# JanWosnitza/FrayTracer

Hardware: AMD Instinct MI355X
Metric: Mrays/s (primary+secondary) at 4096x4096; max per-pixel |delta| vs F# ref (delta is measured against the CPU oracle: F# parity is unpinned, DESIGN.md section 2) (higher is better)
Workload: dtype f32

## Files before the change

fraytracer_amd/_lib.py:

```python
import ctypes as C
import os

_HERE = os.path.dirname(os.path.abspath(__file__))
LIB_PATH = os.environ.get("FRAYTRACER_HIP_LIB") or os.path.join(_HERE, "libfraytracer_hip.so")

FT_OPT_REFILL_MIN, FT_OPT_MAX_BLOCKS_PER_CU, FT_OPT_HOST_CHUNKS, FT_OPT_HOST_PIN, FT_OPT_TAIL_K, FT_OPT_MATH, FT_OPT_GUIDED, FT_OPT_CHUNK, FT_OPT_CULL, FT_OPT_ESCAPE, FT_OPT_LAZY_UNION, FT_OPT_CARVED, FT_OPT_REUSE, FT_OPT_CERT, FT_OPT_CERT_POLICY, FT_OPT_ORDER, FT_OPT_OCCL, FT_OPT_OCCL_POLICY = 1, 2, 3, 4, 5, 6, 7, 8, 9, 10, 11, 12, 13, 14, 15, 16, 17, 18
FT_MATH_FIXED, FT_MATH_GLIBC_FMA, FT_MATH_GLIBC_SSE2 = 0, 1, 2
FT_OK, FT_ERR_INVALID, FT_ERR_NO_DEVICE, FT_ERR_HIP, FT_ERR_UNSUPPORTED, FT_ERR_EMPTY, FT_ERR_COMM = 0, -1, -2, -3, -4, -5, -6


class FrayTracerError(RuntimeError):
    def __init__(self, code, message):
        super().__init__(f"libfraytracer_hip error {code}: {message}")
        self.code = code


class Vec3(C.Structure):
    _fields_ = [("x", C.c_float), ("y", C.c_float), ("z", C.c_float)]


class Ray(C.Structure):
    _fields_ = [("origin", Vec3), ("direction", Vec3), ("length", C.c_float), ("epsilon", C.c_float)]


class Boundary(C.Structure):
    _fields_ = [("center", Vec3), ("radius", C.c_float)]


class Sphere(C.Structure):
# ... 245 lines not shown
```

fraytracer_amd/api.py:

```python
import contextlib
import ctypes as C
import threading

import numpy as np

from . import _lib
from ._lib import lib, check, FrayTracerError


def _v3(v):
    x, y, z = (float(np.float32(c)) for c in v)
    return (x, y, z)


class FColor(tuple):

    @staticmethod
    def ofRGB(r, g, b):
        return FColor(_v3((r, g, b)))


class _Desc:
    __slots__ = ("kind", "args", "kids", "__weakref__")

# ... 337 lines not shown
    @contextlib.contextmanager
    def on_current_stream(self, tensor):
        import torch
        cur = torch.cuda.current_stream(tensor.device)
        side = None
        if int(cur.cuda_stream) == 0:
            side = self._side_stream = getattr(self, "_side_stream", None) or torch.cuda.Stream(tensor.device)
            side.wait_stream(cur)
        handle = int((side or cur).cuda_stream)
        if getattr(self, "_adopted", None) != handle:
            self.set_stream(handle)
        try:
            yield
        finally:
            if side is not None:
                cur.wait_stream(side)

    OPTIONS = {"refill_min": _lib.FT_OPT_REFILL_MIN, "max_blocks_per_cu": _lib.FT_OPT_MAX_BLOCKS_PER_CU,
               "host_chunks": _lib.FT_OPT_HOST_CHUNKS, "host_pin": _lib.FT_OPT_HOST_PIN, "math": _lib.FT_OPT_MATH,
               "tail_k": _lib.FT_OPT_TAIL_K, "guided": _lib.FT_OPT_GUIDED, "chunk": _lib.FT_OPT_CHUNK, "cull": _lib.FT_OPT_CULL, "escape": _lib.FT_OPT_ESCAPE, "lazy_union": _lib.FT_OPT_LAZY_UNION, "carved": _lib.FT_OPT_CARVED, "reuse": _lib.FT_OPT_REUSE,
               "cert": _lib.FT_OPT_CERT, "cert_policy": _lib.FT_OPT_CERT_POLICY,
               "order": _lib.FT_OPT_ORDER,
               "occl": _lib.FT_OPT_OCCL, "occl_policy": _lib.FT_OPT_OCCL_POLICY}

    def set_option(self, name, value):
        check(lib.ft_ctx_set_option(self._ctx, self._option_id(name), int(value)))

    def get_option(self, name):
        v = C.c_int32()
        check(lib.ft_ctx_get_option(self._ctx, self._option_id(name), C.byref(v)))
        return int(v.value)

    def _option_id(self, name):
        return self.OPTIONS[name]

    def sphere(self, c, r): return check(lib.ft_form_sphere(self._ctx, C.byref(_lib.Sphere(_vec(c), r))))
    def capsule(self, a, b, r): return check(lib.ft_form_capsule(self._ctx, C.byref(_lib.Capsule(_vec(a), _vec(b), r))))
    def torus(self, c, n, R, r): return check(lib.ft_form_torus(self._ctx, C.byref(_lib.Torus(_vec(c), _vec(n), R, r))))
    def triangle(self, a, b, c, r): return check(lib.ft_form_triangle(self._ctx, C.byref(_lib.Triangle(_vec(a), _vec(b), _vec(c), r))))
    def box(self, c, h): return check(lib.ft_form_box(self._ctx, C.byref(_lib.Box(_vec(c), _vec(h)))))
    def form_union(self, hs): return check(lib.ft_form_union(self._ctx, *_handles(hs)))
    def form_subtract(self, a, b): return check(lib.ft_form_subtract(self._ctx, a, b))
    def form_intersect(self, hs): return check(lib.ft_form_intersect(self._ctx, *_handles(hs)))
    def form_union_smooth(self, k, hs): return check(lib.ft_form_union_smooth(self._ctx, k, *_handles(hs)))
    def material_solid(self, rgb): return check(lib.ft_material_solid(self._ctx, _f3(rgb)))
    def material_glass(self, tint, ior, dispersion): return check(lib.ft_material_glass(self._ctx, _f3(tint), ior, dispersion))
    def object_create(self, m, f): return check(lib.ft_object_create(self._ctx, m, f))
    def object_union(self, hs): return check(lib.ft_object_union(self._ctx, *_handles(hs)))
    def object_subtract(self, o, f): return check(lib.ft_object_subtract(self._ctx, o, f))
    def object_intersect(self, o, hs): return check(lib.ft_object_intersect(self._ctx, o, *_handles(hs)))
    def light_directional(self, d, c): return check(lib.ft_light_directional(self._ctx, _f3(d), _f3(c)))
    def light_point(self, p, c): return check(lib.ft_light_point(self._ctx, _f3(p), _f3(c)))

    def form_boundary(self, h):
        b = _lib.Boundary()
        check(lib.ft_form_boundary(self._ctx, h, C.byref(b)))
        return (b.center.x, b.center.y, b.center.z, b.radius)
# ... 1042 lines not shown
```

fraytracer_amd/csrc/capi.cpp:

```cpp
#include <hip/hip_runtime_api.h>

#include <algorithm>
#include <atomic>
#include <array>
#include <cmath>
#include <cstdlib>
#include <cstring>
#include <string>
#include <vector>

#include "../../include/fraytracer_hip.h"
#include "build_hash.h"
#include "ft_kernels.h"
#include "ft_mesh.h"
#include "ft_slice.h"
#include "ft_refine.h"
#include "ft_shells.h"
#include "ft_measure.h"
#include "scene.hpp"

#ifndef FT_BUILD_KIND
#define FT_BUILD_KIND "product"
#endif

// ... 29 lines not shown
    std::vector<hipEvent_t> syncEvents;
    std::vector<std::pair<void*, size_t>> hostRegs;
    std::vector<std::pair<hipEvent_t, hipEvent_t>> events;
    std::vector<std::pair<hipEvent_t, hipEvent_t>> eventPool;
    double foldedMs = 0.0;
    int optRefillMin = 64;
    int optMaxBlocksPerCU = 0;
    int optHostChunks = 0;
    int optHostPin = 1;
    int optMath = FT_MATH_FIXED;
    int optTailK = -1;
    int optChunk = 64;
    int optEscape = 1;
    int optLazyUnion = 1;
    int optCull = 1;
    int optReuse = 1;
    int optCarved = 1;
    int optCert = 1;
    int optCertPolicy = 0;
    int optGuided = 0;
    int optOccl = 1;
    int optOcclPolicy = 0;
    int optOrder = 1;
    int fieldBrick = -1;
    uint32_t meshTile = FT_MESH_TILE_DEFAULT;
    uint32_t sliceTile = FT_SLICE_TILE_DEFAULT;
    int sliceStop = 0;
    int64_t sliceLast[2] = {0, 0};
    void* sliceWork = nullptr; size_t sliceWorkBytes = 0;
    void* refineWork = nullptr; size_t refineWorkBytes = 0;
    uint32_t shellsTile = FT_SHELLS_TILE_DEFAULT;
    int shellsStop = 0;
    int64_t shellsLast[2] = {0, 0};
    void* shellsWork = nullptr; size_t shellsWorkBytes = 0;
    void* measureWork = nullptr; size_t measureWorkBytes = 0;
    int measureStop = 0, measureEager = 0;
    unsigned measureGrid = 0;
    int refineSkipField = 0;
    uint32_t orderNum = 1, orderDen = 1;
};

struct TileOrderKey {
    int32_t W, H, x0, nCols;
    uint32_t stripeW, stripeRanks, stripeRank, nJobs, variant, libm;
    bool operator==(const TileOrderKey& o) const {
        return W == o.W && H == o.H && x0 == o.x0 && nCols == o.nCols && stripeW == o.stripeW && stripeRanks == o.stripeRanks && stripeRank == o.stripeRank &&
               nJobs == o.nJobs && variant == o.variant && libm == o.libm;
    }
};
struct TileOrderSlot {
    uint32_t* cost = nullptr; uint32_t* order = nullptr; void* work = nullptr;
    uint32_t capTiles = 0;
    bool keyed = false, hasOrder = false;
    bool usedOrder = false;
    TileOrderKey key{};
};

struct ft_scene {
    ft_ctx* ctx = nullptr;
    ft::FlatScene flat;
    void* dBlob = nullptr;
    FtSceneDev dev{};
    const float* dMaterialsExt = nullptr;
    const int32_t* dMatHandles = nullptr;
    FtCarve carve{};
    bool usesExpLog = false;
    mutable TileOrderSlot orderSlots[2];
};

namespace {

int requireDevice(ft_ctx* c) {
    if (!c) return setErr(FT_ERR_INVALID, "null context");
    if (!c->hasDevice) return setErr(FT_ERR_NO_DEVICE, "context has no GPU: libfraytracer_hip has no CPU fallback");
    hipError_t e = hipSetDevice(c->device);
    if (e != hipSuccess) return hipFail(e, "hipSetDevice");
// ... 155 lines not shown
    hipEvent_t e0, e1;
    if ((rc = acquireEvents(c, e0, e1))) return rc;
    const char* at = "hipEventRecord";
    hipError_t e = hipEventRecord(e0, stream);
    if (e == hipSuccess && (e = launch()) != hipSuccess) at = what;
    if (e == hipSuccess) e = hipEventRecord(e1, stream);
    if (e != hipSuccess) { c->eventPool.emplace_back(e0, e1); return hipFail(e, at); }
    c->events.emplace_back(e0, e1);
    return FT_OK;
}

int clampPerCU(const ft_ctx* c, const char* kernel, int& perCU) {
    if (perCU < 1) return setErr(FT_ERR_UNSUPPORTED, std::string("the ") + kernel + " kernel does not fit a compute unit with this scene's LDS footprint");
    perCU = std::min(perCU, 8);
    if (c->optMaxBlocksPerCU > 0) perCU = std::min(perCU, c->optMaxBlocksPerCU);
    return FT_OK;
}

TileOrderSlot* tileOrderSlot(const ft_scene* s, int lane, uint32_t nTiles) {
    TileOrderSlot& t = s->orderSlots[lane];
    if (t.capTiles >= nTiles) return &t;
    if (t.cost) (void)hipFree(t.cost);
    t = TileOrderSlot{};
    const size_t words = 2 * (size_t)nTiles, bytes = align256(words * sizeof(uint32_t)) + ft_tile_order_work_bytes(nTiles);
    void* p = nullptr;
    if (hipMalloc(&p, bytes) != hipSuccess) { (void)hipGetLastError(); return nullptr; }
    t.cost = static_cast<uint32_t*>(p);
    t.order = t.cost + nTiles;
    t.work = static_cast<unsigned char*>(p) + align256(words * sizeof(uint32_t));
    t.capTiles = nTiles;
    return &t;
}


int gridSize(const ft_ctx* c, const FtTraceKey& key, const KernelPlan& plan, uint32_t nJobs, unsigned& blocks) {
    int perCU = 0;
    HIP_TRY(ft_trace_occupancy(key, plan.lds, &perCU));
    int rc = clampPerCU(c, "trace", perCU); if (rc) return rc;
    if (c->optMaxBlocksPerCU <= 0 && key.variant != 1u) {
        const uint64_t tiles = ((uint64_t)nJobs + (uint64_t)c->optChunk - 1) / (uint64_t)c->optChunk;
        const uint64_t wavesPerLayer = (uint64_t)c->numCUs * (FT_BLOCK / 64);
        const uint64_t want = (tiles + 2 * wavesPerLayer) / (4 * wavesPerLayer);
        perCU = (int)std::min<uint64_t>((uint64_t)perCU, std::max<uint64_t>(2, want));
    }
    const uint64_t maxBlocks = (uint64_t)c->numCUs * perCU;
    const uint64_t wantBlocks = ((uint64_t)nJobs + FT_BLOCK - 1) / FT_BLOCK;
    blocks = (unsigned)std::max<uint64_t>(1, std::min(maxBlocks, wantBlocks));
    return FT_OK;
}

void handOut(const ft_ctx* c, const ft_scene* s, unsigned variant, unsigned blocks, FtRenderArgs& a) {
// ... 23 lines not shown
    a.bundlePeriod = pol.bundle == 0u ? FT_BUNDLE_PERIOD : pol.bundle == 3u ? 0u : pol.bundle;
    a.bundleMin = pol.bundle == 0u ? FT_BUNDLE_MIN : 1u;
    a.bundleShadow = pol.bundle == 0u ? FT_BUNDLE_SHADOW : pol.bundle == 2u ? 2u : 0u;
    if (c->optCertPolicy == 0 && a.cert && a.mode == 0u && a.views == nullptr && a.maxSize > 0.0f) {
        const float* cm = a.cam;
        const double dx = (double)cm[0] - f.hdr.escC[0], dy = (double)cm[1] - f.hdr.escC[1], dz = (double)cm[2] - f.hdr.escC[2];
        auto len = [cm](int i) { return std::sqrt((double)cm[i] * cm[i] + (double)cm[i + 1] * cm[i + 1] + (double)cm[i + 2] * cm[i + 2]); };
        const double up = len(6), rt = len(9), fw = len(3);
        const double reach = std::sqrt(dx * dx + dy * dy + dz * dz) + (double)f.hdr.escR;
        const double tile = 8.0 * std::max(up, rt) / (double)a.maxSize * reach / fw;
        if (fw > 0.0 && tile <= (double)f.hdr.certM) a.certPrim = a.certShadow = 0xffffffffu;
    }
}

void occlSchedule(const ft_ctx* c, const ft::FlatScene& f, FtRenderArgs& a) {
    const OcclPolicy pol = decodeOcclPolicy((uint32_t)c->optOcclPolicy);
    const bool on = a.cert && c->optOccl && f.occ.b >= 0.0f && pol.period != 255u;
    a.occPeriod = on ? (pol.period != 0u ? pol.period : FT_OCCL_PERIOD) : 0u;
    a.occFrom = pol.from + a.reuse;
    a.occMin = pol.minLanes != 0u ? pol.minLanes : FT_OCCL_MIN;
    a.occ = f.occ;
}

TileOrderSlot* tileOrder(const ft_ctx* c, const ft_scene* s, int lane, const FtTraceKey& key, FtRenderArgs& a) {
    a.tileCost = nullptr; a.tileOrder = nullptr;
    TileOrderSlot* slot = nullptr;
    if (key.form == FT_FORM_FRAME && !key.ext && key.variant == 1u && a.mode == 0u && a.spp == 1u && a.chunk == 64u && a.refillMin == 64u && !c->optGuided && a.shrink1 == a.nJobs && a.nJobs >= 64u) {
        if (c->optOrder == 0) { s->orderSlots[lane].keyed = s->orderSlots[lane].hasOrder = s->orderSlots[lane].usedOrder = false; }
        else slot = tileOrderSlot(s, lane, a.nJobs >> 6);
    }
    if (slot) {
        const TileOrderKey k{a.W, a.H, a.x0, a.nCols, a.stripeW, a.stripeRanks, a.stripeRank, a.nJobs, key.variant, key.libm ? 1u : 0u};
        a.tileCost = slot->cost;
        if (c->optOrder == 1 && slot->keyed && slot->hasOrder && slot->key == k) a.tileOrder = slot->order;
        slot->key = k; slot->keyed = true; slot->hasOrder = false; slot->usedOrder = a.tileOrder != nullptr;
    }
    return slot;
}

int launchTrace(ft_ctx* c, const ft_scene* s, FtRenderArgs& a, int lane = 0) {
    hipStream_t stream = lane ? c->lane1 : c->stream;
    uint32_t* counter = c->dCounter + (lane ? 16 : 0);
    KernelPlan plan;
    int rc = planTrace(c, s, a.ext != 0u, a.shade, plan); if (rc) return rc;
    a.S = s->dev; a.S.fastPath = plan.variant; a.S.nSlots = plan.nSlots;
    a.S.mathFma = c->optMath == FT_MATH_GLIBC_FMA ? 1u : 0u;
    if (!c->optEscape) a.S.escR = -1.0f;
    a.carve = s->carve; a.materialsExt = s->dMaterialsExt;
    a.math = plan.libm ? 1u : 0u;
    a.counter = counter; a.stats = c->dStats;
    a.cull = (s->dev.cullPc != 0xffffffffu && plan.cullRows && c->optCull) ? 1u : 0u;
    a.lazy = c->optLazyUnion ? 1u : 0u;
    a.reuse = (c->optReuse && !a.shade) ? 1u : 0u;
    const FtTraceKey key = ft_trace_key(a);
    unsigned blocks = 0;
    if ((rc = gridSize(c, key, plan, a.nJobs, blocks))) return rc;
    handOut(c, s, plan.variant, blocks, a);
    certSchedule(c, s->flat, plan.variant, a);
// ... 8 lines not shown
    return FT_OK;
}

struct OptionSpec { int32_t id; int ft_ctx::*field; int32_t lo, hi; const char* err; };
constexpr OptionSpec kOptions[] = {
    {FT_OPT_REFILL_MIN, &ft_ctx::optRefillMin, 1, 64, "FT_OPT_REFILL_MIN: 1 .. 64"},
    {FT_OPT_MAX_BLOCKS_PER_CU, &ft_ctx::optMaxBlocksPerCU, 0, 8, "FT_OPT_MAX_BLOCKS_PER_CU: 0 (no cap) .. 8"},
    {FT_OPT_HOST_CHUNKS, &ft_ctx::optHostChunks, 0, 16, "FT_OPT_HOST_CHUNKS: 0 (automatic) .. 16"},
    {FT_OPT_HOST_PIN, &ft_ctx::optHostPin, 0, 1, "FT_OPT_HOST_PIN: 0 or 1"},
    {FT_OPT_TAIL_K, &ft_ctx::optTailK, -1, 64, "FT_OPT_TAIL_K: -1 (default), 0 (off) .. 64"},
    {FT_OPT_MATH, &ft_ctx::optMath, FT_MATH_FIXED, FT_MATH_GLIBC_SSE2, "FT_OPT_MATH: 0 fixed, 1 glibc (FMA build), 2 glibc (SSE2 build)"},
    {FT_OPT_GUIDED, &ft_ctx::optGuided, 0, 1, "FT_OPT_GUIDED: 0 or 1"},
    {FT_OPT_CHUNK, &ft_ctx::optChunk, 16, 64, "FT_OPT_CHUNK: 64, 32 or 16"},
    {FT_OPT_CULL, &ft_ctx::optCull, 0, 1, "FT_OPT_CULL: 0 or 1"},
    {FT_OPT_ESCAPE, &ft_ctx::optEscape, 0, 1, "FT_OPT_ESCAPE: 0 or 1"},
    {FT_OPT_LAZY_UNION, &ft_ctx::optLazyUnion, 0, 1, "FT_OPT_LAZY_UNION: 0 or 1"},
    {FT_OPT_CARVED, &ft_ctx::optCarved, 0, 1, "FT_OPT_CARVED: 0 or 1"},
    {FT_OPT_REUSE, &ft_ctx::optReuse, 0, 1, "FT_OPT_REUSE: 0 or 1"},
    {FT_OPT_CERT, &ft_ctx::optCert, 0, 1, "FT_OPT_CERT: 0 or 1"},
    {FT_OPT_CERT_POLICY, &ft_ctx::optCertPolicy, INT32_MIN, INT32_MAX, "FT_OPT_CERT_POLICY: 0, or bits 16-23 (due lanes) in 1 .. 64"},
    {FT_OPT_ORDER, &ft_ctx::optOrder, 0, 2, "FT_OPT_ORDER: 0 off, 1 heavy tiles first, 2 record only"},
    {FT_OPT_OCCL, &ft_ctx::optOccl, 0, 1, "FT_OPT_OCCL: 0 or 1"},
    {FT_OPT_OCCL_POLICY, &ft_ctx::optOcclPolicy, 0, 0x40ffff, "FT_OPT_OCCL_POLICY: 0, or bits 0-7 period, 8-15 first step, 16-23 candidates (0 .. 64)"},
};
const OptionSpec* findOption(int32_t id) {
    for (const OptionSpec& o : kOptions) if (o.id == id) return &o;
    return nullptr;
}
bool optionAccepts(const OptionSpec& o, int32_t v) {
    if (v < o.lo || v > o.hi) return false;
    if (o.id == FT_OPT_CHUNK) return v == 64 || v == 32 || v == 16;
    if (o.id == FT_OPT_CERT_POLICY) { const uint32_t mn = decodeCertPolicy((uint32_t)v).minLanes; return v == 0 || (mn >= 1u && mn <= 64u); }
    return true;
}

int checkJobCount(uint64_t views, uint64_t samples, const ft_render_params* p) {
    const uint64_t tiles = (uint64_t)((p->n_columns + 7) / 8) * (uint64_t)((p->height + 7) / 8);
    if (views * samples * tiles * 64 >= 0xFFFF0000ull) return setErr(FT_ERR_UNSUPPORTED, "more than 2^32 samples in one call");
    return FT_OK;
}

int checkParams(const ft_render_params* p) {
    if (!p) return setErr(FT_ERR_INVALID, "null render params");
    if (p->width <= 0 || p->height <= 0 || p->n_columns <= 0) return setErr(FT_ERR_INVALID, "empty image");
    if (p->stripe_width <= 0 || p->stripe_ranks <= 0 || p->stripe_rank < 0 || p->stripe_rank >= p->stripe_ranks)
        return setErr(FT_ERR_INVALID, "bad stripe description");
// ... 215 lines not shown
    *out = s;
    return FT_OK;
}

void ft_scene_destroy(ft_scene* s) {
    if (!s) return;
    if (s->dBlob) { (void)hipSetDevice(s->ctx->device); (void)hipFree(s->dBlob); }
    for (TileOrderSlot& t : s->orderSlots) if (t.cost) { (void)hipSetDevice(s->ctx->device); (void)hipFree(t.cost); }
    delete s;
}

static long long readTileOrderSlot(const ft_scene* s, bool order, uint32_t* out, long long cap) {
    if (!s || !s->ctx || (!out && cap > 0) || cap < 0) return setErr(FT_ERR_INVALID, "bad argument");
    int rc = requireDevice(s->ctx); if (rc) return rc;
    const TileOrderSlot& t = s->orderSlots[0];
    if (!t.keyed || (order && !t.hasOrder)) return 0;
    const long long n = (long long)(t.key.nJobs >> 6);
    HIP_TRY(hipStreamSynchronize(s->ctx->stream));
    if (std::min(n, cap) > 0) HIP_TRY(hipMemcpy(out, order ? t.order : t.cost, (size_t)std::min(n, cap) * sizeof(uint32_t), hipMemcpyDeviceToHost));
    return n;
}
long long ft_scene_tile_costs(const ft_scene* s, uint32_t* out, long long cap) { return readTileOrderSlot(s, false, out, cap); }
long long ft_scene_tile_order(const ft_scene* s, uint32_t* out, long long cap) { return readTileOrderSlot(s, true, out, cap); }
int ft_scene_tile_order_used(const ft_scene* s) { return s && s->orderSlots[0].keyed && s->orderSlots[0].usedOrder ? 1 : 0; }
int ft_ctx_tile_order_rule(ft_ctx* c, uint32_t num, uint32_t den) {
    if (!c || den == 0u || num > 1000000u || den > 16u) return setErr(FT_ERR_INVALID, "bad argument");
    c->orderNum = num; c->orderDen = den;
    return FT_OK;
}

float ft_lens_create(float fov) { return ft::lensCreate(fov); }
int ft_camera_look_at(const float pos[3], const float look[3], const float up[3], float nps, ft_camera* out) {
    if (!pos || !look || !up || !out) return setErr(FT_ERR_INVALID, "null argument");
    f3 o[4];
    ft::cameraLookAt(tof3(pos), tof3(look), tof3(up), nps, o);
    out->position = ft_vec3{o[0].x, o[0].y, o[0].z}; out->forward = ft_vec3{o[1].x, o[1].y, o[1].z};
    out->up_scaled = ft_vec3{o[2].x, o[2].y, o[2].z}; out->right_scaled = ft_vec3{o[3].x, o[3].y, o[3].z};
    return FT_OK;
}

namespace {

struct Outputs {
    void* rgb; void* hits; void* material;
    bool any() const { return rgb || hits || material; }
    bool extra() const { return hits || material; }
// ... 1836 lines not shown
```

fraytracer_amd/csrc/ft_kernels.h:

```cpp
#pragma once
#include <hip/hip_runtime_api.h>
#include <stddef.h>
#include <stdint.h>

#include "../../include/fraytracer_hip.h"
#include "ft_device.h"
#include "ft_libm.h"

#define FT_BLOCK 256
#define FT_LDS_CNT_WORDS 64
#define FT_LDS_TILE_WORD 40
#define FT_LDS_WAVE_WORD 48
#define FT_LDS_REPORT_WORD 36
static_assert(FT_LDS_WAVE_WORD >= FT_LDS_TILE_WORD + 2 * (256 / 64) && FT_LDS_WAVE_WORD + 4 * (256 / 64) <= FT_LDS_CNT_WORDS, "the wave sums lie behind the tile words, inside the header");
static_assert(FT_LDS_TILE_WORD >= 36 && FT_LDS_TILE_WORD + 2 * (256 / 64) <= FT_LDS_CNT_WORDS, "the tile words lie behind the clocks, inside the header");
#ifdef FT_UNION_PROFILE
#define FT_LDS_DBG_ROWS 13
#else
#define FT_LDS_DBG_ROWS 0
#endif
#define FT_SH_ROWS 10
#define FT_LDS_SH_BASE (FT_LDS_CNT_WORDS + FT_LDS_DBG_ROWS * FT_BLOCK)
#define FT_LDS_HDR_FLOATS (FT_LDS_SH_BASE + FT_SH_ROWS * FT_BLOCK)
#define FT_CULL_MAX 256
#define FT_CULL_ROW (4 * FT_CULL_MAX)

struct FtLdsLayout { uint32_t slotD, slotL, consts, libmTab, rows, total; };
FT_HD FtLdsLayout ft_lds_layout(uint32_t nSlots, uint32_t nStage, bool libm, bool rows) {
    FtLdsLayout L;
    L.slotD = FT_LDS_HDR_FLOATS;
    L.slotL = FT_LDS_HDR_FLOATS + nSlots * FT_BLOCK;
    L.consts = FT_LDS_HDR_FLOATS + 2u * nSlots * FT_BLOCK;
    L.libmTab = (L.consts + nStage + 1u) & ~1u;
    const uint32_t end = libm ? L.libmTab + 2u * FT_LIBM_TAB_DOUBLES : L.consts + nStage;
    L.rows = (end + 3u) & ~3u;
    L.total = rows ? L.rows + FT_CULL_ROW * (FT_BLOCK / 64) : end;
    return L;
}
// ... 21 lines not shown
    uint32_t shrink1, shrink2;
    uint32_t tailK;
    const float* materialsExt;
    float spec[16][4];
    uint32_t reuse;
    FtCarve carve;
    float* hitsOut;
    int32_t* matOut;
    const int32_t* matHandles;
    uint32_t hits;
    uint32_t cert, certPrim, certShadow, certMin, certRepeat;
    const float* views;
    uint32_t nViews;
    uint32_t shade;
    const float* hitsIn;
    uint32_t visSel, visKeep;
    const uint32_t* visIn;
    uint32_t* visOut;
    uint32_t bundlePeriod, bundleMin, bundleShadow;
    uint32_t* tileCost;
    const uint32_t* tileOrder;
    uint32_t occPeriod, occFrom, occMin;
    FtOccl occ;
};
static_assert(offsetof(FtRenderArgs, occ) == 860 && sizeof(FtRenderArgs) == 888, "the kernels' argument block does not move");
#define FT_MAX_VIEWS 64

enum { FT_FORM_FRAME = 0, FT_FORM_VIEWS = 1, FT_FORM_SHADE = 2, FT_FORM_VIS = 3, FT_FORM_NONE = 4 };
FT_HD uint32_t ft_trace_form(bool views, unsigned shade) {
    if (shade) return (views || shade > 2u) ? FT_FORM_NONE : (shade == 2u ? FT_FORM_VIS : FT_FORM_SHADE);
    return views ? FT_FORM_VIEWS : FT_FORM_FRAME;
}
struct FtTraceKey { uint32_t variant, carveKind, form; bool ext, libm; };
FT_HD FtTraceKey ft_trace_key(const FtRenderArgs& a) {
    return FtTraceKey{a.S.fastPath, a.carve.kind, ft_trace_form(a.views != nullptr, a.shade), a.ext != 0u, a.math != 0u};
}

struct FtFieldArgs {
    FtSceneDev S;
    FtCarve carve;
    const float* pts;
    float origin[3], step[3];
    uint32_t ny, nz, nx;
    uint32_t bricksJ, bricksK;
    uint32_t lgJ, lgK;
    uint32_t nJobs;
    uint32_t n;
    uint32_t cull;
// ... 58 lines not shown
```

fraytracer_amd/csrc/kernels.hip:

```cpp
#include <hip/hip_runtime.h>

#include "../../include/fraytracer_hip.h"
#include "ft_device.h"
#include "ft_kernels.h"
#include "ft_math.h"
#include "ft_libm.h"

#define FT_CONST __attribute__((address_space(4)))
typedef const float FT_CONST* cfp;
template <class T> __device__ __forceinline__ const T FT_CONST* as_const(const T* p) {
    return (const T FT_CONST*)(p);
}

__device__ __forceinline__ f3 ld3(cfp c) { return mk3(c[0], c[1], c[2]); }
__device__ __forceinline__ FtInstr ld_instr(const FtInstr FT_CONST* q) {
    FtInstr r; r.op = q->op; r.dst = q->dst; r.src = q->src; r.type = q->type; r.count = q->count; r.data = q->data;
    r.aux = q->aux; r.flags = q->flags; r.f0 = q->f0; r.f1 = q->f1; r.pad0 = 0; r.pad1 = 0; return r;
}
typedef float v4f __attribute__((ext_vector_type(4)));
typedef uint32_t v4u __attribute__((ext_vector_type(4)));
struct ItemRegs { v4f a; v4u b; };
__device__ __forceinline__ ItemRegs ld_item(const FtItemRec FT_CONST* q) {
    ItemRegs r;
    r.a = *reinterpret_cast<const v4f FT_CONST*>(q);
// ... 1484 lines not shown
        s.dir = ft_normalize(D + N * (2.0f * cosi));
        s.o = hp + N * (2.0f * s.eps);
    } else {
        s.dir = ft_normalize(D * eta + N * (eta * cosi - cost));
        s.o = hp - N * (4.0f * s.eps);
        s.xs ^= 0x80000000u;
        if (s.inside()) { cfp t = as_const(a.S.materials) + 3u * s.leaf; s.thr = s.thr * mk3(t[0], t[1], t[2]); }
    }
    s.xs += 0x10000u;
    s.len = a.length; s.steps = 0;
    s.phase = PH_MARCH; s.certAt = a.certPrim;
}

__device__ __forceinline__ void ft_wave_word_add(uint32_t* word, uint32_t v) {
    if ((threadIdx.x & 63u) == 0u) __hip_atomic_fetch_add(word, v, __ATOMIC_RELAXED, __HIP_MEMORY_SCOPE_WORKGROUP);
}

__device__ __forceinline__ unsigned long long wave_sum(uint32_t v) {
    unsigned long long x = v;
    for (int off = 32; off > 0; off >>= 1) x += __shfl_down(x, off, 64);
    return x;
}

template <int VARIANT, bool EXT, int MATH = 0, int K = 0, int FORM = FT_FORM_FRAME>
__device__ __forceinline__ void ft_trace_body(const FtRenderArgs& a) {
    constexpr bool VIEWS = FORM == FT_FORM_VIEWS, SHADE = FORM == FT_FORM_SHADE || FORM == FT_FORM_VIS;
    static_assert(!SHADE || !EXT, "ft_shade_hits and ft_light_visibility have no EXTENSION build");
    constexpr bool LEAN = VARIANT == 1 && !EXT;
    const uint32_t tid = threadIdx.x, lane = tid & 63u;
    unsigned long long* clk0 = reinterpret_cast<unsigned long long*>(ft_lds + 32);
    if (blockIdx.x == 0 && tid == 0) { clk0[0] = clock64(); clk0[1] = wall_clock64(); }
    const FtLdsLayout L = ft_lds_layout(a.S.nSlots, a.S.nStage, MATH != 0, true);
    float* sd = ft_lds + L.slotD + tid;
    uint32_t* sl = reinterpret_cast<uint32_t*>(ft_lds + L.slotL) + tid;
    float* ldsC = ft_lds + L.consts;
    for (uint32_t i = tid; i < a.S.nStage; i += FT_BLOCK) ldsC[i] = a.S.consts[i];
    if (MATH != 0 && tid < FT_LIBM_TAB_DOUBLES) const_cast<ft_u64*>(ft_libm_tab(a.S))[tid] = ft_libm_tab_g[tid];
    if (tid < 32u || (LEAN && (tid - FT_LDS_WAVE_WORD < 4u * (FT_BLOCK / 64) || tid == FT_LDS_REPORT_WORD))) reinterpret_cast<uint32_t*>(ft_lds)[tid] = 0u;
#ifdef FT_UNION_PROFILE
    for (uint32_t k = 0; k < FT_LDS_DBG_ROWS; ++k) reinterpret_cast<uint32_t*>(ft_lds)[FT_LDS_CNT_WORDS + tid + k * FT_BLOCK] = 0u;
#endif
    __syncthreads();
    if (LEAN && blockIdx.x == 0 && tid == 0) reinterpret_cast<uint32_t*>(ft_lds)[FT_LDS_REPORT_WORD] = 1u;

    float* coopRow = ft_lds + ft_lds_layout(a.S.nSlots, a.S.nStage, MATH != 0, true).rows + (uint32_t)__builtin_amdgcn_readfirstlane((int)(tid >> 6)) * FT_CULL_ROW;
    uint32_t cullSkipped = 0, cullTotal = 0;
    uint32_t chunkNext = 0, chunkEnd = 0;
    uint32_t waveEvals = 0;
    constexpr bool ORDER = FORM == FT_FORM_FRAME && !EXT && VARIANT == 1;
    uint32_t* tileSt = reinterpret_cast<uint32_t*>(ft_lds) + FT_LDS_TILE_WORD + (tid >> 6);
    constexpr uint32_t TILE_EVALS = FT_BLOCK / 64;
    if (ORDER && lane == 0) tileSt[0] = 0xffffffffu;
    uint32_t coopEvals = 0;
    uint32_t nEvals = 0;
    uint32_t* waveSt = reinterpret_cast<uint32_t*>(ft_lds) + FT_LDS_WAVE_WORD + (tid >> 6);
    enum : uint32_t { ST_EVALS = 0, ST_COOP = FT_BLOCK / 64, ST_CULL_TOTAL = 2 * (FT_BLOCK / 64), ST_CULL_SKIPPED = 3 * (FT_BLOCK / 64) };
    bool exhausted = false;
    LaneState s;
    s.phase = PH_IDLE; s.job = 0; s.steps = 0; s.lidx = 0; s.leaf = 0; s.outIdx = 0; s.certAt = 0xffffffffu;
    s.o = s.dir = mk3(0, 0, 0);
    s.len = 0; s.eps = 0;
    s.xs = 0;
    s.thr = splat3(1.0f); s.seed = 0;
    bool camKnown = false;
    float dCam = 0.0f; uint32_t leafCam = 0u;
    if (!SHADE && a.reuse != 0u && a.mode == 0u) {
        s.phase = PH_CAM;
        if (VIEWS) { const float* c = a.views + 12u * (lane % a.nViews); s.o = mk3(c[0], c[1], c[2]); }
        else s.o = mk3(a.cam[0], a.cam[1], a.cam[2]);
        s.eps = a.eps;
    }
    ViewCam vc{};

    for (;;) {
        for (int round = 0; round < 3; ++round) {
            const unsigned long long idle = __ballot(s.phase == PH_IDLE);
            if (idle == 0ull) break;
            if ((uint32_t)__popcll(idle) < a.refillMin && __ballot(s.phase >= PH_MARCH) != 0ull) break;
            if (chunkNext == chunkEnd) {
                if (exhausted) break;
                const FtRenderArgs& u = FT_ARGS_AT_USE(LEAN, a);
                if (ORDER && u.tileCost != nullptr && lane == 0) {
                    const uint32_t t = tileSt[0];
                    if (t < (u.nJobs >> 6)) u.tileCost[t] = waveEvals - tileSt[TILE_EVALS];
                    tileSt[0] = 0xffffffffu;
                }
                uint32_t base = 0, take = u.chunk;
                if (lane == 0) {
                    if (u.shrink1 < u.nJobs) {
                        const uint32_t cur = __hip_atomic_load(u.counter, __ATOMIC_RELAXED, __HIP_MEMORY_SCOPE_AGENT);
                        take = cur >= u.shrink2 ? u.chunk / 4u : (cur >= u.shrink1 ? u.chunk / 2u : u.chunk);
                    }
                    base = atomicAdd(u.counter, take);
                }
                base = __builtin_amdgcn_readfirstlane(base);
                const uint32_t took = (uint32_t)__builtin_amdgcn_readfirstlane((int)take);
                if (base >= u.nJobs) { exhausted = true; break; }
                chunkNext = base;
                chunkEnd = (u.nJobs - base < took) ? u.nJobs : base + took;
                if (ORDER && u.tileCost != nullptr) {
                    uint32_t tile = base >> 6;
                    if (u.tileOrder != nullptr) {
                        tile = (uint32_t)__builtin_amdgcn_readfirstlane((int)u.tileOrder[tile]);
                        chunkNext = tile << 6; chunkEnd = chunkNext + 64u;
                    }
                    if (lane == 0) { tileSt[0] = tile; tileSt[TILE_EVALS] = waveEvals; }
                }
            }
            uint32_t avail = chunkEnd - chunkNext;
            if (VIEWS && a.mode == 0u) {
                const uint32_t jobsPerView = a.jobsPerPlane * (EXT ? a.spp : 1u);
                const uint32_t v = chunkNext / jobsPerView, viewEnd = (v + 1u) * jobsPerView;
                if (viewEnd - chunkNext < avail) avail = viewEnd - chunkNext;
                cfp c = as_const(a.views) + 12u * v;
                vc.o = ld3(c); vc.fw = ld3(c + 3); vc.up = ld3(c + 6); vc.rt = ld3(c + 9);
                vc.d = ft_readlane_f(dCam, (int)v); vc.leaf = (uint32_t)__builtin_amdgcn_readlane((int)leafCam, (int)v);
            }
            const uint32_t nIdle = (uint32_t)__popcll(idle);
            const uint32_t rank = (uint32_t)__popcll(idle & ((1ull << lane) - 1ull));
            if (s.phase == PH_IDLE && rank < avail) { s.job = chunkNext + rank; start_job<EXT, FORM, LEAN>(a, s, camKnown, dCam, leafCam, vc); }
            chunkNext += (nIdle < avail) ? nIdle : avail;
        }
        if (s.phase == PH_IDLE && exhausted && chunkNext == chunkEnd) s.phase = PH_DONE;
        if (__ballot(s.phase != PH_DONE) == 0ull) break;

        if (VARIANT == 1 && FT_WORD_AT_USE(LEAN, a.occPeriod) != 0u && waveEvals % a.occPeriod == 0u) {
            const bool cand = s.phase == PH_SHADOW && s.steps - a.occFrom < a.occPeriod && (!EXT || !s.inside());
            if ((uint32_t)__popcll(__ballot(cand)) >= a.occMin) {
                const bool hit = ft_occlusion_certificate<LEAN>(FT_ARGS_AT_USE(LEAN, a), ldsC + 0, cand, s.o, s.dir, s.eps, s.len, s.steps);
                if (hit) { ft_count(FT_C_HITS); s.lidx += 1; s.phase = PH_LIGHTS; settle<EXT, FORM, LEAN>(a, s); }
                if (__ballot(hit) != 0ull && __ballot(s.phase >= PH_MARCH) == 0ull) continue;
            }
        }

        if (VARIANT == 1 && FT_WORD_AT_USE(LEAN, a.cert) != 0u) {
            bool ends = false;
            if (FT_WORD_AT_USE(LEAN, a.bundlePeriod) != 0u && waveEvals % a.bundlePeriod == 0u) {
#pragma unroll 1
                for (uint32_t ph = SHADE ? PH_SHADOW : PH_MARCH; ph <= PH_SHADOW; ph += PH_SHADOW - PH_MARCH) {
                    const bool cand = s.phase == ph && (ph == PH_MARCH || s.steps >= a.bundleShadow) && (!EXT || !s.inside());
                    if ((uint32_t)__popcll(__ballot(cand)) < a.bundleMin) continue;
                    if (ft_bundle_certificate<LEAN>(FT_ARGS_AT_USE(LEAN, a).S, ldsC + 0, cand, s.o, s.dir, s.eps, s.len, s.steps, a.bundleMin)) ends = true;
                }
            }
            const bool due = !ends && (s.phase == PH_MARCH || s.phase == PH_SHADOW) && s.steps >= s.certAt && (!EXT || !s.inside());
            bool tried = false;
            if ((uint32_t)__popcll(__ballot(due)) >= a.certMin) {
                tried = true;
                const FtRenderArgs& u = FT_ARGS_AT_USE(LEAN, a);
                const bool holds = ft_miss_certificate(u.S, ldsC + 0, due, s.o, s.dir, s.eps, s.len, s.steps);
                if (due) {
                    if (holds) ends = true;
                    else s.certAt = u.certRepeat != 0u ? s.steps + u.certRepeat : 0xffffffffu;
                }
            }
            if (ends) { s.len = -1.0f; settle<EXT, FORM, LEAN>(a, s); }
            if ((tried || __ballot(ends) != 0ull) && __ballot(s.phase >= PH_MARCH) == 0ull) continue;
        }

        const bool active = s.phase >= PH_MARCH;
        waveEvals += 1;
        FT_UDBG_T0(tRound);
        auto query_point = [&]() {
            f3 q = s.o;
            if (!SHADE && s.phase >= PH_NX && s.phase <= PH_NC) {
// ... 929 lines not shown
```

include/fraytracer_hip.h:

```cpp
#ifndef FRAYTRACER_HIP_H
#define FRAYTRACER_HIP_H

#include <stdint.h>

#ifdef __cplusplus
extern "C" {
#endif

#define FT_ABI_VERSION 5
#define FT_FIELD_BOUNDED 1u

typedef enum ft_status {
    FT_OK = 0,
    FT_ERR_INVALID = -1,
    FT_ERR_NO_DEVICE = -2,
    FT_ERR_HIP = -3,
    FT_ERR_UNSUPPORTED = -4,
    FT_ERR_EMPTY = -5,
    FT_ERR_COMM = -6
} ft_status;

typedef int32_t ft_handle;
typedef struct ft_ctx ft_ctx;
typedef struct ft_scene ft_scene;
// ... 42 lines not shown
int ft_ctx_create(int device, ft_ctx** out);
void ft_ctx_destroy(ft_ctx* ctx);
const char* ft_last_error(void);
int ft_ctx_set_stream(ft_ctx* ctx, void* hip_stream);
const char* ft_build_info(void);
typedef enum ft_option {
    FT_OPT_REFILL_MIN = 1,
    FT_OPT_MAX_BLOCKS_PER_CU = 2,
    FT_OPT_HOST_CHUNKS = 3,
    FT_OPT_HOST_PIN = 4,
    FT_OPT_TAIL_K = 5,
    FT_OPT_MATH = 6,
    FT_OPT_CHUNK = 8,
    FT_OPT_CULL = 9,
    FT_OPT_ESCAPE = 10,
    FT_OPT_LAZY_UNION = 11,
    FT_OPT_CARVED = 12,
    FT_OPT_REUSE = 13,
    FT_OPT_CERT = 14,
    FT_OPT_CERT_POLICY = 15,
    FT_OPT_ORDER = 16,
    FT_OPT_OCCL = 17,
    FT_OPT_OCCL_POLICY = 18,
    FT_OPT_GUIDED = 7
} ft_option;
typedef enum ft_math_mode { FT_MATH_FIXED = 0, FT_MATH_GLIBC_FMA = 1, FT_MATH_GLIBC_SSE2 = 2 } ft_math_mode;
int ft_ctx_set_option(ft_ctx* ctx, int32_t option, int32_t value);
int ft_ctx_get_option(const ft_ctx* ctx, int32_t option, int32_t* value);

ft_handle ft_form_sphere(ft_ctx*, const ft_sphere*);
ft_handle ft_form_capsule(ft_ctx*, const ft_capsule*);
ft_handle ft_form_torus(ft_ctx*, const ft_torus*);
ft_handle ft_form_triangle(ft_ctx*, const ft_triangle*);
ft_handle ft_form_box(ft_ctx*, const ft_box*);
ft_handle ft_form_union(ft_ctx*, const ft_handle* forms, int32_t n);
ft_handle ft_form_subtract(ft_ctx*, ft_handle a, ft_handle b);
ft_handle ft_form_intersect(ft_ctx*, const ft_handle* forms, int32_t n);
ft_handle ft_form_union_smooth(ft_ctx*, float strength, const ft_handle* forms, int32_t n);
int ft_form_boundary(ft_ctx*, ft_handle form, ft_boundary* out);

ft_handle ft_material_solid(ft_ctx*, const float rgb[3]);
ft_handle ft_material_glass(ft_ctx*, const float tint[3], float ior, float dispersion);
int ft_spectral_table(int32_t nw, float* out);
ft_handle ft_object_create(ft_ctx*, ft_handle material, ft_handle form);
ft_handle ft_object_union(ft_ctx*, const ft_handle* objects, int32_t n);
ft_handle ft_object_subtract(ft_ctx*, ft_handle object, ft_handle form);
// ... 164 lines not shown
```

Before: 1231.

## Schedule bundle certificate tries per tile from the previous frame's hits

Records, per 64-pixel tile, the first wave round at which a bundle miss certificate succeeded for primary and shadow rays, and stores it in a device hint buffer. On the next frame with the same tile layout and a small camera shift, waves try the bundle certificate around the recorded round and at sparse intervals instead of on a fixed period. This aims to cut wasted certificate attempts and end rays sooner, at the cost of extra LDS bookkeeping, a larger argument block, and cross-frame state that only pays off for repeated, near-static renders.

```diff
diff --git a/fraytracer_amd/_lib.py b/fraytracer_amd/_lib.py
--- a/fraytracer_amd/_lib.py
+++ b/fraytracer_amd/_lib.py
@@ -4,7 +4,7 @@
 _HERE = os.path.dirname(os.path.abspath(__file__))
 LIB_PATH = os.environ.get("FRAYTRACER_HIP_LIB") or os.path.join(_HERE, "libfraytracer_hip.so")
 
-FT_OPT_REFILL_MIN, FT_OPT_MAX_BLOCKS_PER_CU, FT_OPT_HOST_CHUNKS, FT_OPT_HOST_PIN, FT_OPT_TAIL_K, FT_OPT_MATH, FT_OPT_GUIDED, FT_OPT_CHUNK, FT_OPT_CULL, FT_OPT_ESCAPE, FT_OPT_LAZY_UNION, FT_OPT_CARVED, FT_OPT_REUSE, FT_OPT_CERT, FT_OPT_CERT_POLICY, FT_OPT_ORDER, FT_OPT_OCCL, FT_OPT_OCCL_POLICY = 1, 2, 3, 4, 5, 6, 7, 8, 9, 10, 11, 12, 13, 14, 15, 16, 17, 18
+FT_OPT_REFILL_MIN, FT_OPT_MAX_BLOCKS_PER_CU, FT_OPT_HOST_CHUNKS, FT_OPT_HOST_PIN, FT_OPT_TAIL_K, FT_OPT_MATH, FT_OPT_GUIDED, FT_OPT_CHUNK, FT_OPT_CULL, FT_OPT_ESCAPE, FT_OPT_LAZY_UNION, FT_OPT_CARVED, FT_OPT_REUSE, FT_OPT_CERT, FT_OPT_CERT_POLICY, FT_OPT_ORDER, FT_OPT_OCCL, FT_OPT_OCCL_POLICY, FT_OPT_TRY_HINT = 1, 2, 3, 4, 5, 6, 7, 8, 9, 10, 11, 12, 13, 14, 15, 16, 17, 18, 19
 FT_MATH_FIXED, FT_MATH_GLIBC_FMA, FT_MATH_GLIBC_SSE2 = 0, 1, 2
 FT_OK, FT_ERR_INVALID, FT_ERR_NO_DEVICE, FT_ERR_HIP, FT_ERR_UNSUPPORTED, FT_ERR_EMPTY, FT_ERR_COMM = 0, -1, -2, -3, -4, -5, -6
 
diff --git a/fraytracer_amd/api.py b/fraytracer_amd/api.py
--- a/fraytracer_amd/api.py
+++ b/fraytracer_amd/api.py
@@ -383,6 +383,7 @@
                "cert": _lib.FT_OPT_CERT, "cert_policy": _lib.FT_OPT_CERT_POLICY,
                "order": _lib.FT_OPT_ORDER,
                "occl": _lib.FT_OPT_OCCL, "occl_policy": _lib.FT_OPT_OCCL_POLICY}
+    STREAM_OPTIONS = {"try_hint": _lib.FT_OPT_TRY_HINT}
 
     def set_option(self, name, value):
         check(lib.ft_ctx_set_option(self._ctx, self._option_id(name), int(value)))
@@ -393,7 +394,7 @@
         return int(v.value)
 
     def _option_id(self, name):
-        return self.OPTIONS[name]
+        return self.OPTIONS[name] if name in self.OPTIONS else self.STREAM_OPTIONS[name]
 
     def sphere(self, c, r): return check(lib.ft_form_sphere(self._ctx, C.byref(_lib.Sphere(_vec(c), r))))
     def capsule(self, a, b, r): return check(lib.ft_form_capsule(self._ctx, C.byref(_lib.Capsule(_vec(a), _vec(b), r))))
diff --git a/fraytracer_amd/csrc/capi.cpp b/fraytracer_amd/csrc/capi.cpp
--- a/fraytracer_amd/csrc/capi.cpp
+++ b/fraytracer_amd/csrc/capi.cpp
@@ -75,6 +75,7 @@
     int optOccl = 1;
     int optOcclPolicy = 0;
     int optOrder = 1;
+    int optTryHint = 1;
     int fieldBrick = -1;
     uint32_t meshTile = FT_MESH_TILE_DEFAULT;
     uint32_t sliceTile = FT_SLICE_TILE_DEFAULT;
@@ -102,9 +103,11 @@
     }
 };
 struct TileOrderSlot {
-    uint32_t* cost = nullptr; uint32_t* order = nullptr; void* work = nullptr;
+    uint32_t* cost = nullptr; uint32_t* order = nullptr; uint32_t* hint = nullptr; void* work = nullptr;
     uint32_t capTiles = 0;
     bool keyed = false, hasOrder = false;
+    float hintCam[12] = {};
+    bool hasHint = false, usedHint = false; TileOrderKey hintKey{};
     bool usedOrder = false;
     TileOrderKey key{};
 };
@@ -306,11 +309,12 @@
     if (t.capTiles >= nTiles) return &t;
     if (t.cost) (void)hipFree(t.cost);
     t = TileOrderSlot{};
-    const size_t words = 2 * (size_t)nTiles, bytes = align256(words * sizeof(uint32_t)) + ft_tile_order_work_bytes(nTiles);
+    const size_t words = 3 * (size_t)nTiles, bytes = align256(words * sizeof(uint32_t)) + ft_tile_order_work_bytes(nTiles);
     void* p = nullptr;
     if (hipMalloc(&p, bytes) != hipSuccess) { (void)hipGetLastError(); return nullptr; }
     t.cost = static_cast<uint32_t*>(p);
     t.order = t.cost + nTiles;
+    t.hint = t.order + nTiles;
     t.work = static_cast<unsigned char*>(p) + align256(words * sizeof(uint32_t));
     t.capTiles = nTiles;
     return &t;
@@ -380,18 +384,46 @@
     a.occ = f.occ;
 }
 
+constexpr double FT_HINT_MAX_SHIFT = 16.0;
+double cameraShiftPixels(const float* p, const float* q, float maxSize, const ft::FlatScene& f) {
+    auto len = [](const double* v) { return std::sqrt(v[0] * v[0] + v[1] * v[1] + v[2] * v[2]); };
+    double d[4][3], fp[3], fq[3], ec[3];
+    for (int v = 0; v < 4; ++v) for (int i = 0; i < 3; ++i) d[v][i] = (double)q[3 * v + i] - (double)p[3 * v + i];
+    for (int i = 0; i < 3; ++i) { fp[i] = p[3 + i]; fq[i] = q[3 + i]; ec[i] = (double)q[i] - f.hdr.escC[i]; }
+    const double lp = len(fp), lq = len(fq);
+    const double up[3] = {q[6], q[7], q[8]}, rt[3] = {q[9], q[10], q[11]};
+    const double side = std::max(len(up), len(rt));
+    if (!(lp > 0.0) || !(lq > 0.0) || !(side > 0.0) || !(maxSize > 0.0f)) return INFINITY;
+    const double pixel = side / (double)maxSize / lq;
+    const double turn[3] = {fq[0] / lq - fp[0] / lp, fq[1] / lq - fp[1] / lp, fq[2] / lq - fp[2] / lp};
+    const double nearSide = std::max(len(ec) - (double)f.hdr.escR, 0.1 * (double)f.hdr.escR);
+    const double moved = len(d[0]);
+    if (moved > 0.0 && !(nearSide > 0.0)) return INFINITY;
+    const double shift = len(turn) / pixel + (len(d[2]) + len(d[3])) / side * 0.5 * (double)maxSize + (moved > 0.0 ? moved / nearSide / pixel : 0.0);
+    return shift == shift ? shift : INFINITY;
+}
 TileOrderSlot* tileOrder(const ft_ctx* c, const ft_scene* s, int lane, const FtTraceKey& key, FtRenderArgs& a) {
-    a.tileCost = nullptr; a.tileOrder = nullptr;
+    a.tileCost = nullptr; a.tileOrder = nullptr; a.tileHint = nullptr; a.tryHint = 0u;
     TileOrderSlot* slot = nullptr;
     if (key.form == FT_FORM_FRAME && !key.ext && key.variant == 1u && a.mode == 0u && a.spp == 1u && a.chunk == 64u && a.refillMin == 64u && !c->optGuided && a.shrink1 == a.nJobs && a.nJobs >= 64u) {
         if (c->optOrder == 0) { s->orderSlots[lane].keyed = s->orderSlots[lane].hasOrder = s->orderSlots[lane].usedOrder = false; }
-        else slot = tileOrderSlot(s, lane, a.nJobs >> 6);
+        if (c->optTryHint == 0) s->orderSlots[lane].hasHint = false;
+        if (c->optOrder != 0 || c->optTryHint != 0) slot = tileOrderSlot(s, lane, a.nJobs >> 6);
     }
     if (slot) {
         const TileOrderKey k{a.W, a.H, a.x0, a.nCols, a.stripeW, a.stripeRanks, a.stripeRank, a.nJobs, key.variant, key.libm ? 1u : 0u};
         a.tileCost = slot->cost;
-        if (c->optOrder == 1 && slot->keyed && slot->hasOrder && slot->key == k) a.tileOrder = slot->order;
-        slot->key = k; slot->keyed = true; slot->hasOrder = false; slot->usedOrder = a.tileOrder != nullptr;
+        if (c->optOrder != 0) {
+            if (c->optOrder == 1 && slot->keyed && slot->hasOrder && slot->key == k) a.tileOrder = slot->order;
+            slot->key = k; slot->keyed = true; slot->hasOrder = false; slot->usedOrder = a.tileOrder != nullptr;
+        }
+        if (c->optTryHint != 0) {
+            const bool bundleAlone = c->optCertPolicy == 0 && a.cert != 0u && a.bundlePeriod != 0u && a.certPrim == 0xffffffffu && a.certShadow == 0xffffffffu;
+            a.tileHint = slot->hint;
+            if (c->optTryHint == 1 && bundleAlone && slot->hasHint && slot->hintKey == k && cameraShiftPixels(slot->hintCam, a.cam, a.maxSize, s->flat) <= FT_HINT_MAX_SHIFT) a.tryHint = 1u;
+            slot->hintKey = k; slot->hasHint = true; slot->usedHint = a.tryHint != 0u;
+            memcpy(slot->hintCam, a.cam, sizeof(slot->hintCam));
+        }
     }
     return slot;
 }
@@ -446,6 +478,7 @@
     {FT_OPT_ORDER, &ft_ctx::optOrder, 0, 2, "FT_OPT_ORDER: 0 off, 1 heavy tiles first, 2 record only"},
     {FT_OPT_OCCL, &ft_ctx::optOccl, 0, 1, "FT_OPT_OCCL: 0 or 1"},
     {FT_OPT_OCCL_POLICY, &ft_ctx::optOcclPolicy, 0, 0x40ffff, "FT_OPT_OCCL_POLICY: 0, or bits 0-7 period, 8-15 first step, 16-23 candidates (0 .. 64)"},
+    {FT_OPT_TRY_HINT, &ft_ctx::optTryHint, 0, 2, "FT_OPT_TRY_HINT: 0 off, 1 tries scheduled from the last frame, 2 record only"},
 };
 const OptionSpec* findOption(int32_t id) {
     for (const OptionSpec& o : kOptions) if (o.id == id) return &o;
@@ -707,6 +740,39 @@
 }
 long long ft_scene_tile_costs(const ft_scene* s, uint32_t* out, long long cap) { return readTileOrderSlot(s, false, out, cap); }
 long long ft_scene_tile_order(const ft_scene* s, uint32_t* out, long long cap) { return readTileOrderSlot(s, true, out, cap); }
+long long ft_selftest_try_hints(const ft_scene* s, uint32_t* out, long long cap) {
+    if (!s || !s->ctx || (!out && cap > 0) || cap < 0) return setErr(FT_ERR_INVALID, "bad argument");
+    int rc = requireDevice(s->ctx); if (rc) return rc;
+    const TileOrderSlot& t = s->orderSlots[0];
+    if (!t.hasHint) return 0;
+    const long long n = (long long)(t.hintKey.nJobs >> 6);
+    HIP_TRY(hipStreamSynchronize(s->ctx->stream));
+    if (std::min(n, cap) > 0) HIP_TRY(hipMemcpy(out, t.hint, (size_t)std::min(n, cap) * sizeof(uint32_t), hipMemcpyDeviceToHost));
+    return n;
+}
+long long ft_selftest_try_hints_fill(const ft_scene* s, int32_t mode, uint32_t value) {
+    if (!s || !s->ctx || mode < 0 || mode > 1) return setErr(FT_ERR_INVALID, "bad argument");
+    int rc = requireDevice(s->ctx); if (rc) return rc;
+    const TileOrderSlot& t = s->orderSlots[0];
+    if (!t.hasHint) return 0;
+    const size_t n = t.hintKey.nJobs >> 6;
+    std::vector<uint32_t> w(n, value);
+    if (mode == 1) { uint64_t x = value * 2654435761ull + 88172645463325252ull; for (uint32_t& v : w) { x ^= x << 13; x ^= x >> 7; x ^= x << 17; v = (uint32_t)(x >> 24); } }
+    HIP_TRY(hipStreamSynchronize(s->ctx->stream));
+    HIP_TRY(hipMemcpy(t.hint, w.data(), n * sizeof(uint32_t), hipMemcpyHostToDevice));
+    return (long long)n;
+}
+long long ft_selftest_try_hints_write(const ft_scene* s, const uint32_t* words, long long n) {
+    if (!s || !s->ctx || !words) return setErr(FT_ERR_INVALID, "bad argument");
+    int rc = requireDevice(s->ctx); if (rc) return rc;
+    const TileOrderSlot& t = s->orderSlots[0];
+    if (!t.hasHint) return 0;
+    if (n != (long long)(t.hintKey.nJobs >> 6)) return setErr(FT_ERR_INVALID, "not the slot's tile count");
+    HIP_TRY(hipStreamSynchronize(s->ctx->stream));
+    HIP_TRY(hipMemcpy(t.hint, words, (size_t)n * sizeof(uint32_t), hipMemcpyHostToDevice));
+    return n;
+}
+int ft_selftest_try_hints_used(const ft_scene* s) { return s && s->orderSlots[0].hasHint && s->orderSlots[0].usedHint ? 1 : 0; }
 int ft_scene_tile_order_used(const ft_scene* s) { return s && s->orderSlots[0].keyed && s->orderSlots[0].usedOrder ? 1 : 0; }
 int ft_ctx_tile_order_rule(ft_ctx* c, uint32_t num, uint32_t den) {
     if (!c || den == 0u || num > 1000000u || den > 16u) return setErr(FT_ERR_INVALID, "bad argument");
diff --git a/fraytracer_amd/csrc/ft_kernels.h b/fraytracer_amd/csrc/ft_kernels.h
--- a/fraytracer_amd/csrc/ft_kernels.h
+++ b/fraytracer_amd/csrc/ft_kernels.h
@@ -14,6 +14,22 @@
 #define FT_LDS_REPORT_WORD 36
 static_assert(FT_LDS_WAVE_WORD >= FT_LDS_TILE_WORD + 2 * (256 / 64) && FT_LDS_WAVE_WORD + 4 * (256 / 64) <= FT_LDS_CNT_WORDS, "the wave sums lie behind the tile words, inside the header");
 static_assert(FT_LDS_TILE_WORD >= 36 && FT_LDS_TILE_WORD + 2 * (256 / 64) <= FT_LDS_CNT_WORDS, "the tile words lie behind the clocks, inside the header");
+#define FT_LDS_HINT_WORD 24
+static_assert(FT_LDS_HINT_WORD + 2 * (256 / 64) <= 32, "the hint words lie in the statistics' unused rows");
+
+#define FT_HINT_NONE 255u
+#define FT_HINT_MAX 254u
+#define FT_HINT_USED 0x10000u
+#define FT_HINT_AFTER 2u
+#define FT_HINT_IDLE 4u
+FT_HD uint32_t ft_hint_pack(uint32_t primary, uint32_t shadow) { return (primary & 255u) | (shadow & 255u) << 8; }
+FT_HD uint32_t ft_hint_primary(uint32_t w) { return w & 255u; }
+FT_HD uint32_t ft_hint_shadow(uint32_t w) { return (w >> 8) & 255u; }
+FT_HD uint32_t ft_hint_note(uint32_t w, bool primary, uint32_t r) {
+    const uint32_t v = r < FT_HINT_MAX ? r : FT_HINT_MAX, p = ft_hint_primary(w), s = ft_hint_shadow(w);
+    return primary ? ft_hint_pack(v < p ? v : p, s) : ft_hint_pack(p, v < s ? v : s);
+}
+
 #ifdef FT_UNION_PROFILE
 #define FT_LDS_DBG_ROWS 13
 #else
@@ -81,8 +97,10 @@
     const uint32_t* tileOrder;
     uint32_t occPeriod, occFrom, occMin;
     FtOccl occ;
+    uint32_t* tileHint;
+    uint32_t tryHint, pad1;
 };
-static_assert(offsetof(FtRenderArgs, occ) == 860 && sizeof(FtRenderArgs) == 888, "the kernels' argument block does not move");
+static_assert(offsetof(FtRenderArgs, occ) == 860 && offsetof(FtRenderArgs, tileHint) == 888 && sizeof(FtRenderArgs) == 904, "the kernels' argument block does not move");
 #define FT_MAX_VIEWS 64
 
 enum { FT_FORM_FRAME = 0, FT_FORM_VIEWS = 1, FT_FORM_SHADE = 2, FT_FORM_VIS = 3, FT_FORM_NONE = 4 };
diff --git a/fraytracer_amd/csrc/kernels.hip b/fraytracer_amd/csrc/kernels.hip
--- a/fraytracer_amd/csrc/kernels.hip
+++ b/fraytracer_amd/csrc/kernels.hip
@@ -1530,6 +1530,13 @@
     return x;
 }
 
+__device__ __forceinline__ bool ft_try_due(uint32_t h, uint32_t n, uint32_t r) {
+    if (r % FT_HINT_IDLE == 0u) return true;
+    if (h != FT_HINT_NONE && (r + 1u == h || r == h)) return true;
+    const uint32_t from = n != FT_HINT_NONE ? n : h;
+    return from != FT_HINT_NONE && r > from && (r - from) % FT_HINT_AFTER == 0u;
+}
+
 template <int VARIANT, bool EXT, int MATH = 0, int K = 0, int FORM = FT_FORM_FRAME>
 __device__ __forceinline__ void ft_trace_body(const FtRenderArgs& a) {
     constexpr bool VIEWS = FORM == FT_FORM_VIEWS, SHADE = FORM == FT_FORM_SHADE || FORM == FT_FORM_VIS;
@@ -1559,6 +1566,8 @@
     uint32_t* tileSt = reinterpret_cast<uint32_t*>(ft_lds) + FT_LDS_TILE_WORD + (tid >> 6);
     constexpr uint32_t TILE_EVALS = FT_BLOCK / 64;
     if (ORDER && lane == 0) tileSt[0] = 0xffffffffu;
+    uint32_t* hintSt = reinterpret_cast<uint32_t*>(ft_lds) + FT_LDS_HINT_WORD + (tid >> 6);
+    constexpr uint32_t HINT_NOTE = FT_BLOCK / 64;
     uint32_t coopEvals = 0;
     uint32_t nEvals = 0;
     uint32_t* waveSt = reinterpret_cast<uint32_t*>(ft_lds) + FT_LDS_WAVE_WORD + (tid >> 6);
@@ -1590,7 +1599,10 @@
                 const FtRenderArgs& u = FT_ARGS_AT_USE(LEAN, a);
                 if (ORDER && u.tileCost != nullptr && lane == 0) {
                     const uint32_t t = tileSt[0];
-                    if (t < (u.nJobs >> 6)) u.tileCost[t] = waveEvals - tileSt[TILE_EVALS];
+                    if (t < (u.nJobs >> 6)) {
+                        u.tileCost[t] = waveEvals - tileSt[TILE_EVALS];
+                        if (u.tileHint != nullptr) u.tileHint[t] = hintSt[HINT_NOTE];
+                    }
                     tileSt[0] = 0xffffffffu;
                 }
                 uint32_t base = 0, take = u.chunk;
@@ -1612,7 +1624,11 @@
                         tile = (uint32_t)__builtin_amdgcn_readfirstlane((int)u.tileOrder[tile]);
                         chunkNext = tile << 6; chunkEnd = chunkNext + 64u;
                     }
-                    if (lane == 0) { tileSt[0] = tile; tileSt[TILE_EVALS] = waveEvals; }
+                    if (lane == 0) {
+                        tileSt[0] = tile; tileSt[TILE_EVALS] = waveEvals;
+                        hintSt[0] = u.tryHint != 0u ? (u.tileHint[tile] & 0xffffu) | FT_HINT_USED : 0u;
+                        hintSt[HINT_NOTE] = ft_hint_pack(FT_HINT_NONE, FT_HINT_NONE);
+                    }
                 }
             }
             uint32_t avail = chunkEnd - chunkNext;
@@ -1643,12 +1659,18 @@
 
         if (VARIANT == 1 && FT_WORD_AT_USE(LEAN, a.cert) != 0u) {
             bool ends = false;
-            if (FT_WORD_AT_USE(LEAN, a.bundlePeriod) != 0u && waveEvals % a.bundlePeriod == 0u) {
+            const uint32_t hint = ORDER ? (uint32_t)__builtin_amdgcn_readfirstlane((int)hintSt[0]) : 0u;
+            const uint32_t noted = ORDER ? (uint32_t)__builtin_amdgcn_readfirstlane((int)hintSt[HINT_NOTE]) : 0u;
+            const uint32_t tileRound = ORDER ? waveEvals - (uint32_t)__builtin_amdgcn_readfirstlane((int)tileSt[TILE_EVALS]) : 0u;
+            if (FT_WORD_AT_USE(LEAN, a.bundlePeriod) != 0u && ((ORDER && hint != 0u) || waveEvals % a.bundlePeriod == 0u)) {
 #pragma unroll 1
                 for (uint32_t ph = SHADE ? PH_SHADOW : PH_MARCH; ph <= PH_SHADOW; ph += PH_SHADOW - PH_MARCH) {
+                    if (ORDER && hint != 0u && !ft_try_due(ph == PH_MARCH ? ft_hint_primary(hint) : ft_hint_shadow(hint), ph == PH_MARCH ? ft_hint_primary(noted) : ft_hint_shadow(noted), tileRound)) continue;
                     const bool cand = s.phase == ph && (ph == PH_MARCH || s.steps >= a.bundleShadow) && (!EXT || !s.inside());
                     if ((uint32_t)__popcll(__ballot(cand)) < a.bundleMin) continue;
-                    if (ft_bundle_certificate<LEAN>(FT_ARGS_AT_USE(LEAN, a).S, ldsC + 0, cand, s.o, s.dir, s.eps, s.len, s.steps, a.bundleMin)) ends = true;
+                    const bool held = ft_bundle_certificate<LEAN>(FT_ARGS_AT_USE(LEAN, a).S, ldsC + 0, cand, s.o, s.dir, s.eps, s.len, s.steps, a.bundleMin);
+                    if (held) ends = true;
+                    if (ORDER && __ballot(held) != 0ull && lane == 0) hintSt[HINT_NOTE] = ft_hint_note(hintSt[HINT_NOTE], ph == PH_MARCH, tileRound);
                 }
             }
             const bool due = !ends && (s.phase == PH_MARCH || s.phase == PH_SHADOW) && s.steps >= s.certAt && (!EXT || !s.inside());
diff --git a/include/fraytracer_hip.h b/include/fraytracer_hip.h
--- a/include/fraytracer_hip.h
+++ b/include/fraytracer_hip.h
@@ -88,6 +88,7 @@
     FT_OPT_ORDER = 16,
     FT_OPT_OCCL = 17,
     FT_OPT_OCCL_POLICY = 18,
+    FT_OPT_TRY_HINT = 19,
     FT_OPT_GUIDED = 7
 } ft_option;
 typedef enum ft_math_mode { FT_MATH_FIXED = 0, FT_MATH_GLIBC_FMA = 1, FT_MATH_GLIBC_SSE2 = 2 } ft_math_mode;
```

Result: faster. 1252, median of 6 (+1.7%).
